# flxrcz/hommx

Hardware: AMD Instinct MI355X
Metric: micro-cell solves/sec (higher is better)
Workload: dtype f64

## Files before the change

### hommx_amd/csrc/fused2d.hip

```cpp
#include <hip/hip_runtime.h>
#include <stdint.h>

#include "kernels.h"
#include "sweep_acc.h"

#ifndef HOMMX_FUSED_WAVES_PER_SIMD
#define HOMMX_FUSED_WAVES_PER_SIMD 2
#endif

namespace hommx {

typedef double d4 __attribute__((ext_vector_type(4)));
typedef double d2 __attribute__((ext_vector_type(2)));

__device__ __forceinline__ double uniform_f64(double v) {
  return __hiloint2double(__builtin_amdgcn_readfirstlane(__double2hiint(v)),
                          __builtin_amdgcn_readfirstlane(__double2loint(v)));
}

struct CoefRow {
  double a0, a1;
  double a0m, a1m;
};

constexpr int MATP = 48;

template <int NB>
struct alignas(16) Lds {
  double mat[(NB + 1) * MATP];
  double ubuf[4 * NB];
  double tsc[16 * 17];
  double rrow[2][NB];
  double vrow[2][NB];
  double vnat[2][NB];
  double e0row[NB];
  double e1row[NB];
  double e0nat[NB];
  double e1nat[NB];
  double dgnat[NB];
  double cenat[NB + 2];
};

template <int NB>
__global__ __launch_bounds__(64, HOMMX_FUSED_WAVES_PER_SIMD) void k_poisson2d_fused(
    const double* __restrict__ coef, const double* __restrict__ Mmat, double* __restrict__ out,
    int32_t* __restrict__ info, int n, long long ncells, const CoefSource src
#ifdef HOMMX_FUSED_DEBUG
    , double* __restrict__ dbg
#endif
) {
  constexpr int NT = NB / 16, KK = NB / 4, CG = 64 / NB;
  constexpr int P = MATP;
  __shared__ Lds<NB> L;

  const long long cell = blockIdx.x;
  if (cell >= ncells) return;
  __builtin_assume(n >= 3);
  __builtin_assume(n <= NB);
  const int l = threadIdx.x;
  const int j = l & 15, k = l >> 4;
  const int c = l % NB, g = l / NB;
  const int lb = l - c;
  const int p0 = NB - n;
  const bool valid = c >= p0;
  const int cn = c - p0;
  const int cm = valid ? (c == p0 ? NB - 1 : c - 1) : c;
  const int cp = valid ? (c == NB - 1 ? p0 : c + 1) : c;
  const int prow = (c & 3) * KK + (c >> 2);

  const int ownB = (k + 1) * P + j;
  int leftB[NT];
#pragma unroll
  for (int tj = 0; tj < NT; ++tj) {
    const int col = 16 * tj + j;
    leftB[tj] = (k + 1) * P + (col == p0 ? NB - 1 : col - 1);
  }
#define OWN(ti, tj, r) (ownB + (16 * (ti) + 4 * (r)) * P + 16 * (tj))
#define LEFT(ti, tj, r) (leftB[tj] + (16 * (ti) + 4 * (r)) * P)
  const unsigned matOff = accl::lds_offset(&L.mat[0]);
  const unsigned haloA = matOff + 8u * (unsigned)(p0 * P + j);

  for (int i = l; i < (NB + 1) * P; i += 64) L.mat[i] = 0.0;
  if (l == 0) L.cenat[0] = 0.0;

  double m00 = 1.0, m01 = 0.0, m10 = 0.0, m11 = 1.0;
  if (Mmat) {
    const double* mp = Mmat + cell * 4;
    m00 = mp[0]; m01 = mp[1]; m10 = mp[2]; m11 = mp[3];
  }
// ... 79 lines not shown
    {
      const double dv = st_diag(rowB, rowA), ov = st_E(rowB, rowA);
      band_write(dv, ov, true, false);
      __syncthreads();
#pragma unroll
      for (int ti = 0; ti < NT; ++ti)
#pragma unroll
        for (int tj = 0; tj <= ti; ++tj)
#pragma unroll
          for (int r = 0; r < 4; ++r) slr[ti][tj][r] = L.mat[OWN(ti, tj, r)];
      __syncthreads();
      band_write(dv, ov, true, true);
      __syncthreads();
    }
    {
      const double dv = st_N(rowB), ov = st_NE(rowB);
      band_write(dv, ov, false, false);
      __syncthreads();
#pragma unroll
      for (int t = 0; t < NT; ++t)
#pragma unroll
        for (int kk = 0; kk < KK; ++kk) wf[t][kk] = L.mat[OWN(kk >> 2, t, kk & 3)];
      __syncthreads();
      band_write(dv, ov, false, true);
      __syncthreads();
    }
    {
      const double dv = -st_diag(cur, rowB), ov = -st_E(cur, rowB);
      band_write(dv, ov, true, false);
      __syncthreads();
#pragma unroll
      for (int ti = 0; ti < NT; ++ti)
#pragma unroll
        for (int tj = 0; tj < NT; ++tj)
#pragma unroll
          for (int r = 0; r < 4; ++r) a[ti][tj][r] = L.mat[OWN(ti, tj, r)];
      __syncthreads();
      band_write(dv, ov, true, true);
      __syncthreads();
    }
    rr[0] = st_p0(cur, rowB); rr[1] = st_p1(cur, rowB);
    rlm = (k >> 1) ? st_p1(rowB, rowA) : st_p0(rowB, rowA);
  }
  double ga_ = 0.0, gb_ = 0.0;
  int bad = 0, badstep = 0;
  double wselR[NT];
#pragma unroll
  for (int tj = 0; tj < NT; ++tj) wselR[tj] = (k == 3 && 16 * tj + j == p0) ? 1.0 : 0.0;
  const double wselC = (j == 15 && k == (p0 & 3)) ? 1.0 : 0.0;
  double indw[KK];
#pragma unroll
  for (int q = 0; q < KK; ++q) indw[q] = uniform_f64((q == (p0 >> 2)) ? 1.0 : 0.0);

  for (int jr = 0; jr <= n - 2; ++jr) {
    const bool lastStep = (jr == n - 2);
    CoefRow nxt = cur;
    if (!lastStep) {
      nxt = load_row(jr + 1);
      asum += nxt.a0 + nxt.a1;
    }
    const double e0c = st_N(cur);
    const double neC = st_NE(cur);
    const double e1c = __shfl(neC, lb + cm, 64);
    if (lastStep) {
      for (int i = l; i < (NB + 1) * P; i += 64) L.mat[i] = 0.0;
      __syncthreads();
      if (g == 0) {
        L.mat[(c + 1) * P + c] = e0c;
        if (valid) L.mat[(c + 1) * P + cp] = neC;
      }
      __syncthreads();
#pragma unroll
      for (int t = 0; t < NT; ++t)
#pragma unroll
        for (int kk = 0; kk < KK; ++kk) wf[t][kk] += L.mat[OWN(kk >> 2, t, kk & 3)];
      __syncthreads();
    }
    const double dgc = st_diag(nxt, cur), cec = st_E(nxt, cur);
    if (g == 0) {
      L.rrow[0][prow] = rr[0];
      L.rrow[1][prow] = rr[1];
      L.e0row[prow] = e0c;
      L.e1row[prow] = e1c;
      L.e0nat[c] = e0c;
      L.e1nat[c] = e1c;
      L.dgnat[c] = dgc;
      L.cenat[1 + c] = cec;
    }

    {
      int badj = 0;
#ifdef HOMMX_FUSED_SWEEP32
      accl::Sweep<NB>::run(a, L.ubuf, j, k, badj);
#else
      __builtin_amdgcn_s_setprio(1);
      if constexpr (NB == 32) accl::block_inverse32(a, L.ubuf, L.tsc, j, k, badj);
      else accl::Sweep<NB>::run(a, L.ubuf, j, k, badj);
      __builtin_amdgcn_s_setprio(0);
#endif
      if (badj && !bad) { bad = 1; badstep = jr + 1; }
    }
#ifdef HOMMX_FUSED_DEBUG
    if (dbg && cell == 0) {
      double* q = dbg + (size_t)jr * 4 * NB * NB;
#pragma unroll
      for (int ti = 0; ti < NT; ++ti)
#pragma unroll
        for (int tj = 0; tj < NT; ++tj)
#pragma unroll
          for (int r = 0; r < 4; ++r) q[(16 * ti + 4 * r + k) * NB + 16 * tj + j] = a[ti][tj][r];
#pragma unroll
      for (int t = 0; t < NT; ++t)
#pragma unroll
        for (int kk = 0; kk < KK; ++kk) q[NB * NB + (16 * t + j) * NB + 4 * kk + k] = wf[t][kk];
    }
#endif

    if (!lastStep) {
#pragma unroll
      for (int ti = 0; ti < NT; ++ti)
#pragma unroll
        for (int tj = 0; tj < NT; ++tj)
#pragma unroll
          for (int r = 0; r < 4; ++r) L.mat[OWN(ti, tj, r)] = a[ti][tj][r];
#pragma unroll
      for (int tj = 0; tj < NT; ++tj)
        accl::masked_lds_store<accl::RowMask<3>::lo, accl::RowMask<3>::hi>(haloA + 128u * tj, a[NT - 1][tj][3]);
    }

    d4 vt[NT][NT];
#pragma unroll
    for (int x = 0; x < NT; ++x)
#pragma unroll
      for (int y = 0; y < NT; ++y) vt[x][y] = d4{0.0, 0.0, 0.0, 0.0};
#pragma unroll
    for (int kk = 0; kk < KK; ++kk)
#pragma unroll
      for (int x = 0; x < NT; ++x)
#pragma unroll
        for (int y = 0; y < NT; ++y)
          vt[x][y] = __builtin_amdgcn_mfma_f64_16x16x4f64(a[kk >> 2][x][kk & 3], wf[y][kk], vt[x][y], 0, 0, 0);

#pragma unroll
    for (int kk = 0; kk < KK; ++kk)
#pragma unroll
      for (int x = 0; x < NT; ++x)
#pragma unroll
        for (int y = 0; y <= x; ++y)
          slr[x][y] = __builtin_amdgcn_mfma_f64_16x16x4f64(vt[kk >> 2][x][kk & 3], wf[y][kk], slr[x][y], 0, 0, 0);

    double z;
    {
      double part[2][NT];
#pragma unroll
      for (int m = 0; m < 2; ++m)
#pragma unroll
        for (int tj = 0; tj < NT; ++tj) part[m][tj] = 0.0;
#pragma unroll
      for (int m = 0; m < 2; ++m)
#pragma unroll
        for (int ti = 0; ti < NT; ++ti) {
          const d4 q = *reinterpret_cast<const d4*>(&L.rrow[m][k * KK + 4 * ti]);
#pragma unroll
          for (int r = 0; r < 4; ++r)
#pragma unroll
            for (int tj = 0; tj < NT; ++tj) part[m][tj] = fma(q[r], a[ti][tj][r], part[m][tj]);
        }
      if (NT == 2) {
        double s_[2];
#pragma unroll
        for (int m = 0; m < 2; ++m) {
          double x = part[m][0], y = part[m][NT - 1];
          swap16(x, y);
          s_[m] = x + y;
        }
        swap32(s_[0], s_[1]);
        z = s_[0] + s_[1];
      } else {
        double x = part[0][0], y = part[1][0];
        swap32(x, y);
        z = add_xor16(x + y);
      }
    }
    ga_ = fma(z, rr[0], ga_);
    gb_ = fma(z, rr[1], gb_);
    L.vnat[k >> 1][c] = z;
    L.vrow[k >> 1][prow] = z;

    {
      double part[2][NT];
#pragma unroll
      for (int m = 0; m < 2; ++m) {
        double v[KK];
#pragma unroll
        for (int q4 = 0; q4 < KK; q4 += 4) {
          const d4 q = *reinterpret_cast<const d4*>(&L.vrow[m][k * KK + q4]);
          v[q4] = q[0]; v[q4 + 1] = q[1]; v[q4 + 2] = q[2]; v[q4 + 3] = q[3];
        }
#pragma unroll
        for (int t = 0; t < NT; ++t) {
          double acc = 0.0;
#pragma unroll
          for (int kk = 0; kk < KK; ++kk) acc = fma(v[kk], wf[t][kk], acc);
          part[m][t] = acc;
        }
      }
      double z6;
      if (NT == 2) {
        double s_[2];
#pragma unroll
        for (int m = 0; m < 2; ++m) {
          double x = part[m][0], y = part[m][NT - 1];
          swap16(x, y);
          s_[m] = x + y;
        }
        swap32(s_[0], s_[1]);
        z6 = s_[0] + s_[1];
      } else {
        double x = part[0][0], y = part[1][0];
        swap32(x, y);
        z6 = add_xor16(x + y);
      }
      rlm += z6;
    }

    if (!lastStep) {
      double e0r[KK], e1r[KK];
#pragma unroll
      for (int q4 = 0; q4 < KK; q4 += 4) {
        const d4 x = *reinterpret_cast<const d4*>(&L.e0row[k * KK + q4]);
        const d4 y = *reinterpret_cast<const d4*>(&L.e1row[k * KK + q4]);
        e0r[q4] = x[0]; e0r[q4 + 1] = x[1]; e0r[q4 + 2] = x[2]; e0r[q4 + 3] = x[3];
        e1r[q4] = y[0]; e1r[q4 + 1] = y[1]; e1r[q4 + 2] = y[2]; e1r[q4 + 3] = y[3];
      }
      {
        double e0q[NT], e1q[NT], dgq[NT], ceq[NT], cemq[NT];
#pragma unroll
        for (int tj = 0; tj < NT; ++tj) {
          e0q[tj] = L.e0nat[16 * tj + j];
          e1q[tj] = L.e1nat[16 * tj + j];
          dgq[tj] = L.dgnat[16 * tj + j];
          ceq[tj] = L.cenat[1 + 16 * tj + j];
          cemq[tj] = L.cenat[16 * tj + j];
        }
#pragma unroll
        for (int ti = 0; ti < NT; ++ti)
#pragma unroll
          for (int r = 0; r < 4; ++r)
#pragma unroll
            for (int tj = 0; tj < NT; ++tj) {
              const double nl = L.mat[LEFT(ti, tj, r)];
              const double nu = L.mat[OWN(ti, tj, r) - P];
              const double nul = L.mat[LEFT(ti, tj, r) - P];
              const double x = fma(e1q[tj], nl, e0q[tj] * a[ti][tj][r]);
              const double xu = fma(e1q[tj], nul, e0q[tj] * nu);
              a[ti][tj][r] = -fma(e0r[4 * ti + r], x, e1r[4 * ti + r] * xu);
            }
#pragma unroll
        for (int t = 0; t < NT; ++t) {
          using namespace accl;
#define DIAG_LO(r) (OneLane<0, 4 * (r)>::lo | OneLane<1, 4 * (r) + 1>::lo | OneLane<2, 4 * (r) + 2>::lo | OneLane<3, 4 * (r) + 3>::lo)
#define DIAG_HI(r) (OneLane<0, 4 * (r)>::hi | OneLane<1, 4 * (r) + 1>::hi | OneLane<2, 4 * (r) + 2>::hi | OneLane<3, 4 * (r) + 3>::hi)
          masked_sub4<DIAG_LO(0), DIAG_HI(0), DIAG_LO(1), DIAG_HI(1), DIAG_LO(2), DIAG_HI(2), DIAG_LO(3), DIAG_HI(3)>(
              a[t][t][0], a[t][t][1], a[t][t][2], a[t][t][3], dgq[t]);
#define SUB_LO(r) (((r) ? OneLane<0, (4 * (r) - 1) & 15>::lo : 0u) | OneLane<1, 4 * (r)>::lo | OneLane<2, 4 * (r) + 1>::lo | OneLane<3, 4 * (r) + 2>::lo)
#define SUB_HI(r) (((r) ? OneLane<0, (4 * (r) - 1) & 15>::hi : 0u) | OneLane<1, 4 * (r)>::hi | OneLane<2, 4 * (r) + 1>::hi | OneLane<3, 4 * (r) + 2>::hi)
          masked_sub4<SUB_LO(0), SUB_HI(0), SUB_LO(1), SUB_HI(1), SUB_LO(2), SUB_HI(2), SUB_LO(3), SUB_HI(3)>(
              a[t][t][0], a[t][t][1], a[t][t][2], a[t][t][3], ceq[t]);
#define SUP_LO(r) (OneLane<0, 4 * (r) + 1>::lo | OneLane<1, 4 * (r) + 2>::lo | OneLane<2, 4 * (r) + 3>::lo | ((r) < 3 ? OneLane<3, (4 * (r) + 4) & 15>::lo : 0u))
#define SUP_HI(r) (OneLane<0, 4 * (r) + 1>::hi | OneLane<1, 4 * (r) + 2>::hi | OneLane<2, 4 * (r) + 3>::hi | ((r) < 3 ? OneLane<3, (4 * (r) + 4) & 15>::hi : 0u))
          masked_sub4<SUP_LO(0), SUP_HI(0), SUP_LO(1), SUP_HI(1), SUP_LO(2), SUP_HI(2), SUP_LO(3), SUP_HI(3)>(
              a[t][t][0], a[t][t][1], a[t][t][2], a[t][t][3], cemq[t]);
#undef DIAG_LO
#undef DIAG_HI
#undef SUB_LO
#undef SUB_HI
#undef SUP_LO
#undef SUP_HI
        }
        if (NT == 2) {
          using namespace accl;
          masked_sub<OneLane<0, 15>::lo, OneLane<0, 15>::hi>(a[NT - 1][0][0], ceq[0]);
          masked_sub<OneLane<3, 0>::lo, OneLane<3, 0>::hi>(a[0][NT - 1][3], cemq[NT - 1]);
        }
        {
          const double cw = readlane_f64(cec, NB - 1);
#pragma unroll
          for (int tj = 0; tj < NT; ++tj) a[NT - 1][tj][3] = fma(-cw, wselR[tj], a[NT - 1][tj][3]);
          const double vcol = -cw * wselC;
#pragma unroll
          for (int ti = 0; ti < NT; ++ti)
#pragma unroll
            for (int r = 0; r < 4; ++r) a[ti][NT - 1][r] = fma(vcol, indw[4 * ti + r], a[ti][NT - 1][r]);
        }
      }

#pragma unroll
      for (int x = 0; x < NT; ++x)
#pragma unroll
        for (int y = 0; y < NT; ++y)
#pragma unroll
          for (int r = 0; r < 4; ++r) L.mat[OWN(x, y, r)] = vt[x][y][r];
#pragma unroll
      for (int y = 0; y < NT; ++y)
        accl::masked_lds_store<accl::RowMask<3>::lo, accl::RowMask<3>::hi>(haloA + 128u * y, vt[NT - 1][y][3]);
#pragma unroll
      for (int t = 0; t < NT; ++t)
#pragma unroll
        for (int kk = 0; kk < KK; ++kk) {
          const double up = L.mat[OWN(kk >> 2, t, kk & 3) - P];
          wf[t][kk] = fma(e1r[kk], up, e0r[kk] * vt[kk >> 2][t][kk & 3]);
        }

      {
        const double v0 = L.vnat[0][c], v1 = L.vnat[1][c];
        const double vm0 = L.vnat[0][cm], vm1 = L.vnat[1][cm];
        rr[0] = fma(vm0, e1c, fma(v0, e0c, st_p0(nxt, cur)));
        rr[1] = fma(vm1, e1c, fma(v1, e0c, st_p1(nxt, cur)));
      }
      cur = nxt;
      __syncthreads();
    }
  }

  {
    if (NT == 2) {
#pragma unroll
      for (int r = 0; r < 4; ++r) L.mat[OWN(1, 0, r)] = slr[NT - 1][0][r];
      __syncthreads();
    }
#pragma unroll
    for (int ti = 0; ti < NT; ++ti)
#pragma unroll
      for (int tj = 0; tj < NT; ++tj)
#pragma unroll
        for (int r = 0; r < 4; ++r) {
          if (tj <= ti) a[ti][tj][r] = -slr[ti][tj][r];
          else a[ti][tj][r] = -L.mat[(16 + j + 1) * P + 4 * r + k];
        }
    {
      using namespace accl;
#pragma unroll
      for (int tj = 0; tj < NT; ++tj) amov<RowMask<3>::lo, RowMask<3>::hi>(a[NT - 1][tj][3], 0.0);
#pragma unroll
      for (int ti = 0; ti < NT; ++ti)
#pragma unroll
        for (int r = 0; r < 4; ++r) amov<ColMask<15>::lo, ColMask<15>::hi>(a[ti][NT - 1][r], 0.0);
      amov<OneLane<3, 15>::lo, OneLane<3, 15>::hi>(a[NT - 1][NT - 1][3], -1.0);
    }
    if (c == NB - 1) rlm = 0.0;
    __syncthreads();
    L.rrow[k >> 1][prow] = rlm;
    L.vnat[k >> 1][c] = rlm;
    __syncthreads();
    int badj = 0;
    accl::Sweep<NB>::run(a, L.ubuf, j, k, badj);
    if (badj && !bad) { bad = 1; badstep = n; }
    double part[2][NT];
#pragma unroll
    for (int m = 0; m < 2; ++m)
#pragma unroll
      for (int tj = 0; tj < NT; ++tj) part[m][tj] = 0.0;
#pragma unroll
    for (int m = 0; m < 2; ++m)
#pragma unroll
      for (int ti = 0; ti < NT; ++ti) {
        const d4 q = *reinterpret_cast<const d4*>(&L.rrow[m][k * KK + 4 * ti]);
#pragma unroll
        for (int r = 0; r < 4; ++r)
#pragma unroll
          for (int tj = 0; tj < NT; ++tj) part[m][tj] = fma(q[r], a[ti][tj][r], part[m][tj]);
      }
    double z;
    if (NT == 2) {
      double s_[2];
#pragma unroll
// ... 12 lines not shown
    ga_ = fma(z, L.vnat[0][c], ga_);
    gb_ = fma(z, L.vnat[1][c], gb_);
  }

  double g00 = (k < 2) ? ga_ : 0.0, g01 = (k < 2) ? gb_ : 0.0, g11 = (k < 2) ? 0.0 : gb_;
#pragma unroll
  for (int off = 32; off >= 1; off >>= 1) {
    g00 += __shfl_xor(g00, off, 64);
    g01 += __shfl_xor(g01, off, 64);
    g11 += __shfl_xor(g11, off, 64);
    asum += __shfl_xor(asum, off, 64);
  }
  if (l == 0) {
    const double h = 1.0 / n;
    constexpr int DUP = 32 / NB;
    const double sc = 0.25 * h * h / DUP;
    const double c0 = 0.5 * h * h * asum / CG;
    const double t00 = m00 * g00 + m01 * g01, t01 = m00 * g01 + m01 * g11;
    const double t10 = m10 * g00 + m11 * g01, t11 = m10 * g01 + m11 * g11;
    double* o = out + cell * 4;
    o[0] = c0 + sc * (t00 * m00 + t01 * m01);
    o[1] = sc * (t00 * m10 + t01 * m11);
    o[2] = sc * (t10 * m00 + t11 * m01);
    o[3] = c0 + sc * (t10 * m10 + t11 * m11);
    if (info) info[cell] = bad ? badstep : 0;
  }
#undef OWN
#undef LEFT
}

hipError_t launch_poisson2d_fused(const double* d_coef, const double* d_M, double* d_out, int32_t* d_info,
                                  int n, long long ncells, hipStream_t stream, CoefSource src) {
  if (ncells <= 0) return hipSuccess;
  dim3 grid((unsigned)ncells), block(64);
#ifndef HOMMX_DEV_LDS_PAD
#define HOMMX_DEV_LDS_PAD 0
#endif
#ifdef HOMMX_FUSED_DEBUG
  extern double* g_fused_dbg;
  if (n <= 16)
    hipLaunchKernelGGL(k_poisson2d_fused<16>, grid, block, 0, stream, d_coef, d_M, d_out, d_info, n, ncells, src, g_fused_dbg);
  else
    hipLaunchKernelGGL(k_poisson2d_fused<32>, grid, block, 0, stream, d_coef, d_M, d_out, d_info, n, ncells, src, g_fused_dbg);
#else
  if (n <= 16)
    hipLaunchKernelGGL(k_poisson2d_fused<16>, grid, block, HOMMX_DEV_LDS_PAD, stream, d_coef, d_M, d_out, d_info, n, ncells, src);
  else
    hipLaunchKernelGGL(k_poisson2d_fused<32>, grid, block, HOMMX_DEV_LDS_PAD, stream, d_coef, d_M, d_out, d_info, n, ncells, src);
#endif
  return hipGetLastError();
}

}
```

### hommx_amd/csrc/sweep_acc.h

```cpp
#pragma once
#include <hip/hip_runtime.h>
#include <stdint.h>

#include "sweep.h"

namespace hommx {
namespace accl {

template <int K> struct RowMask {
  static constexpr unsigned lo = K == 0 ? 0x0000FFFFu : K == 1 ? 0xFFFF0000u : 0u;
  static constexpr unsigned hi = K == 2 ? 0x0000FFFFu : K == 3 ? 0xFFFF0000u : 0u;
};
template <int J> struct ColMask {
  static constexpr unsigned lo = (1u << J) | (1u << (16 + J));
  static constexpr unsigned hi = lo;
};
template <int K, int J> struct OneLane {
  static constexpr int bit = 16 * K + J;
  static constexpr unsigned lo = bit < 32 ? 1u << (bit & 31) : 0u;
  static constexpr unsigned hi = bit >= 32 ? 1u << (bit & 31) : 0u;
};

#define HOMMX_EXEC_SET(LO, HI) "s_mov_b32 exec_lo, %[" LO "]\n\ts_mov_b32 exec_hi, %[" HI "]\n\t"
#define HOMMX_EXEC_ALL "s_mov_b64 exec, -1"
// ... 18 lines not shown
__device__ __forceinline__ void masked_lds_store(unsigned addr, double v) {
  asm volatile(HOMMX_EXEC_SET("lo", "hi") "ds_write_b64 %[a], %[v]\n\t" HOMMX_EXEC_ALL
               : : [a] "v"(addr), [v] "v"(v), [lo] "i"(LO), [hi] "i"(HI) : "memory");
}
template <unsigned LO, unsigned HI>
__device__ __forceinline__ void masked_lds_store2(unsigned addr0, double v0, unsigned addr1, double v1) {
  asm volatile(HOMMX_EXEC_SET("lo", "hi") "ds_write_b64 %[a0], %[v0]\n\tds_write_b64 %[a1], %[v1]\n\t" HOMMX_EXEC_ALL
               : : [a0] "v"(addr0), [v0] "v"(v0), [a1] "v"(addr1), [v1] "v"(v1), [lo] "i"(LO), [hi] "i"(HI) : "memory");
}
template <unsigned RLO, unsigned RHI>
__device__ __forceinline__ void row_rule2(double& a0, double& a1, double w0, double w1) {
  asm(HOMMX_EXEC_SET("rlo", "rhi") "v_mov_b64 %[a0], %[w0]\n\tv_mov_b64 %[a1], %[w1]\n\t" HOMMX_EXEC_ALL
      : [a0] "+v"(a0), [a1] "+v"(a1) : [w0] "v"(w0), [w1] "v"(w1), [rlo] "i"(RLO), [rhi] "i"(RHI));
}
template <unsigned RLO, unsigned RHI>
__device__ __forceinline__ void row_rule1(double& a0, double w0) {
  asm(HOMMX_EXEC_SET("rlo", "rhi") "v_mov_b64 %[a0], %[w0]\n\t" HOMMX_EXEC_ALL : [a0] "+v"(a0) : [w0] "v"(w0), [rlo] "i"(RLO), [rhi] "i"(RHI));
}
template <int R> struct DiagMask {
  static constexpr unsigned lo = OneLane<0, 4 * R>::lo | OneLane<1, 4 * R + 1>::lo | OneLane<2, 4 * R + 2>::lo | OneLane<3, 4 * R + 3>::lo;
  static constexpr unsigned hi = OneLane<0, 4 * R>::hi | OneLane<1, 4 * R + 1>::hi | OneLane<2, 4 * R + 2>::hi | OneLane<3, 4 * R + 3>::hi;
};
__device__ __forceinline__ void diag_plus_one(double& d0, double& d1, double& d2, double& d3) {
  asm(HOMMX_EXEC_SET("l0", "h0") "v_add_f64 %[d0], %[d0], 1.0\n\t" HOMMX_EXEC_SET("l1", "h1") "v_add_f64 %[d1], %[d1], 1.0\n\t"
      HOMMX_EXEC_SET("l2", "h2") "v_add_f64 %[d2], %[d2], 1.0\n\t" HOMMX_EXEC_SET("l3", "h3") "v_add_f64 %[d3], %[d3], 1.0\n\t"
      HOMMX_EXEC_ALL
      : [d0] "+v"(d0), [d1] "+v"(d1), [d2] "+v"(d2), [d3] "+v"(d3)
      : [l0] "i"(DiagMask<0>::lo), [h0] "i"(DiagMask<0>::hi), [l1] "i"(DiagMask<1>::lo), [h1] "i"(DiagMask<1>::hi),
        [l2] "i"(DiagMask<2>::lo), [h2] "i"(DiagMask<2>::hi), [l3] "i"(DiagMask<3>::lo), [h3] "i"(DiagMask<3>::hi));
}

template <class T>
__device__ __forceinline__ unsigned lds_offset(T* p) {
  return (unsigned)(uintptr_t)(__attribute__((address_space(3))) T*)p;
}

__device__ __forceinline__ double readlane_neg_pivot(double v, int lane, unsigned& mn) {
  const int lo = __builtin_amdgcn_readlane(__double2loint(v), lane);
  const int hi = __builtin_amdgcn_readlane(__double2hiint(v), lane);
  const unsigned t = (unsigned)hi + 0x100000u;
  mn = t < mn ? t : mn;
  return __hiloint2double(hi, lo);
}
__device__ __forceinline__ int bad_pivot_min(unsigned mn) { return mn < 0x80200000u; }

#define HOMMX_BC " row_newbcast:%[jk] row_mask:0xf bank_mask:0xf\n\t"
#define HOMMX_PAIR(X, Y) "v_fmac_f64_dpp %[" Y "], %[" X "], %[wo]" HOMMX_BC "v_fmac_f64_dpp %[" X "], %[" X "], %[wk]" HOMMX_BC
#define HOMMX_ONE(X) "v_fmac_f64_dpp %[" X "], %[" X "], %[wk]" HOMMX_BC
#define HOMMX_RCP0 "v_rcp_f64 %[r], %[d]\n\t"
#define HOMMX_RCPE "v_fma_f64 %[e], -%[d], %[r], 1.0\n\t"
#define HOMMX_RCPT "v_fma_f64 %[e], %[e], %[e], %[e]\n\t"
#define HOMMX_RCPR "v_fma_f64 %[r], %[r], %[e], %[r]\n\t"

template <int NB> struct Sweep;

template <>
struct Sweep<32> {
  static constexpr int NB = 32, NT = 2;
  typedef double Mat[2][2][4];

  template <int K>
  static __device__ __forceinline__ void step(Mat& a, double* ubuf, int lk, int j, unsigned& bad, double u0, double u1, double pinv, int npiv) {
    constexpr int tK = K / 16, jK = K % 16, rK = (K % 16) / 4, kK = K % 4, o = 1 - tK;
    constexpr bool more = K + 1 < NB;
    constexpr int K1 = more ? K + 1 : K;
    constexpr int tK1 = K1 / 16, jK1 = K1 % 16, rK1 = (K1 % 16) / 4, kK1 = K1 % 4;
    constexpr int E = tK1 * 4 + rK1;
#define PI(i) ((i) < E ? (i) : (i) + 1)
#define XR(i) a[PI(i) / 4][tK][PI(i) % 4]
#define YR(i) a[PI(i) / 4][o][PI(i) % 4]
    double w[2];
    w[0] = u0 * -pinv;
    w[1] = u1 * -pinv;
    double nu0 = 0.0, nu1 = 0.0, pn = 1.0;
    if constexpr (more) {
      asm volatile("s_nop 1\n\t" HOMMX_PAIR("x", "y")
                   : [x] "+v"(a[tK1][tK][rK1]), [y] "+v"(a[tK1][o][rK1])
                   : [wk] "v"(w[tK]), [wo] "v"(w[o]), [jk] "n"(jK));
      ubuf[lk + j] = a[tK1][0][rK1];
      ubuf[lk + 16 + j] = a[tK1][1][rK1];
      const double dn = readlane_neg_pivot(a[tK1][tK1][rK1], 16 * kK1 + jK1, bad);
      ubuf[NB * kK1 + K1] = dn - 1.0;
      nu0 = ubuf[NB * kK1 + j];
      nu1 = ubuf[NB * kK1 + 16 + j];
      asm volatile("" ::: "memory");
      double e;
      asm volatile(HOMMX_RCP0 HOMMX_PAIR("x0", "y0") HOMMX_PAIR("x1", "y1") HOMMX_RCPE HOMMX_PAIR("x2", "y2")
                       HOMMX_PAIR("x3", "y3") HOMMX_RCPT HOMMX_PAIR("x4", "y4") HOMMX_PAIR("x5", "y5") HOMMX_RCPR
                           HOMMX_PAIR("x6", "y6")
                   : [x0] "+v"(XR(0)), [y0] "+v"(YR(0)), [x1] "+v"(XR(1)), [y1] "+v"(YR(1)), [x2] "+v"(XR(2)), [y2] "+v"(YR(2)),
                     [x3] "+v"(XR(3)), [y3] "+v"(YR(3)), [x4] "+v"(XR(4)), [y4] "+v"(YR(4)), [x5] "+v"(XR(5)), [y5] "+v"(YR(5)),
                     [x6] "+v"(XR(6)), [y6] "+v"(YR(6)), [r] "=&v"(pn), [e] "=&v"(e)
                   : [wk] "v"(w[tK]), [wo] "v"(w[o]), [d] "s"(dn), [jk] "n"(jK));
    } else {
      asm volatile("s_nop 1\n\t" HOMMX_PAIR("x0", "y0") HOMMX_PAIR("x1", "y1") HOMMX_PAIR("x2", "y2") HOMMX_PAIR("x3", "y3")
                       HOMMX_PAIR("x4", "y4") HOMMX_PAIR("x5", "y5") HOMMX_PAIR("x6", "y6") HOMMX_PAIR("x7", "y7")
                   : [x0] "+v"(a[0][tK][0]), [y0] "+v"(a[0][o][0]), [x1] "+v"(a[0][tK][1]), [y1] "+v"(a[0][o][1]),
                     [x2] "+v"(a[0][tK][2]), [y2] "+v"(a[0][o][2]), [x3] "+v"(a[0][tK][3]), [y3] "+v"(a[0][o][3]),
                     [x4] "+v"(a[1][tK][0]), [y4] "+v"(a[1][o][0]), [x5] "+v"(a[1][tK][1]), [y5] "+v"(a[1][o][1]),
                     [x6] "+v"(a[1][tK][2]), [y6] "+v"(a[1][o][2]), [x7] "+v"(a[1][tK][3]), [y7] "+v"(a[1][o][3])
                   : [wk] "v"(w[tK]), [wo] "v"(w[o]), [jk] "n"(jK));
    }
#undef PI
#undef XR
#undef YR
    row_rule2<RowMask<kK>::lo, RowMask<kK>::hi>(a[tK][0][rK], a[tK][1][rK], w[0], w[1]);
    if constexpr (more) {
      if (K + 1 < npiv) step<K + 1>(a, ubuf, lk, j, bad, nu0, nu1, pn, npiv);
    }
  }

  static __device__ __forceinline__ void run(Mat& a, double* ubuf, int j, int k, int& bad, int npiv = NB) {
    const int lk = NB * k;
    ubuf[lk + j] = a[0][0][0];
    ubuf[lk + 16 + j] = a[0][1][0];
    unsigned b = 0xffffffffu;
    const double d0 = readlane_neg_pivot(a[0][0][0], 0, b);
    ubuf[0] = d0 - 1.0;
    const double u0 = ubuf[j], u1 = ubuf[16 + j];
    step<0>(a, ubuf, lk, j, b, u0, u1, fast_rcp(d0), npiv);
    diag_plus_one(a[0][0][0], a[0][0][1], a[0][0][2], a[0][0][3]);
    diag_plus_one(a[1][1][0], a[1][1][1], a[1][1][2], a[1][1][3]);
    bad |= bad_pivot_min(b);
  }
};

template <>
struct Sweep<16> {
  static constexpr int NB = 16, NT = 1;
  typedef double Mat[1][1][4];

  template <int K>
  static __device__ __forceinline__ void step(Mat& a, double* ubuf, int lk, int j, unsigned& bad, double u0, double pinv, int npiv) {
    constexpr int jK = K, rK = K / 4, kK = K % 4;
    constexpr bool more = K + 1 < NB;
    constexpr int K1 = more ? K + 1 : K;
    constexpr int jK1 = K1, rK1 = K1 / 4, kK1 = K1 % 4;
#define PI(i) ((i) < rK1 ? (i) : (i) + 1)
    const double w = u0 * -pinv;
    double nu0 = 0.0, pn = 1.0;
    if constexpr (more) {
      asm volatile("s_nop 1\n\t" HOMMX_ONE("x") : [x] "+v"(a[0][0][rK1]) : [wk] "v"(w), [jk] "n"(jK));
      ubuf[lk + j] = a[0][0][rK1];
      const double dn = readlane_neg_pivot(a[0][0][rK1], 16 * kK1 + jK1, bad);
      ubuf[NB * kK1 + K1] = dn - 1.0;
      nu0 = ubuf[NB * kK1 + j];
      asm volatile("" ::: "memory");
      double e;
      asm volatile(HOMMX_RCP0 HOMMX_ONE("x0") HOMMX_RCPE HOMMX_ONE("x1") HOMMX_RCPT HOMMX_ONE("x2") HOMMX_RCPR
                   : [x0] "+v"(a[0][0][PI(0)]), [x1] "+v"(a[0][0][PI(1)]), [x2] "+v"(a[0][0][PI(2)]), [r] "=&v"(pn), [e] "=&v"(e)
                   : [wk] "v"(w), [d] "s"(dn), [jk] "n"(jK));
    } else {
      asm volatile("s_nop 1\n\t" HOMMX_ONE("x0") HOMMX_ONE("x1") HOMMX_ONE("x2") HOMMX_ONE("x3")
                   : [x0] "+v"(a[0][0][0]), [x1] "+v"(a[0][0][1]), [x2] "+v"(a[0][0][2]), [x3] "+v"(a[0][0][3])
                   : [wk] "v"(w), [jk] "n"(jK));
    }
#undef PI
#ifdef HOMMX_ROW_RULE_EXEC
    row_rule1<RowMask<kK>::lo, RowMask<kK>::hi>(a[0][0][rK], w);
#else
    a[0][0][rK] = (lk == NB * kK) ? w : a[0][0][rK];
#endif
    if constexpr (more) {
      if (K + 1 < npiv) step<K + 1>(a, ubuf, lk, j, bad, nu0, pn, npiv);
    }
  }

  static __device__ __forceinline__ void run(Mat& a, double* ubuf, int j, int k, int& bad, int npiv = NB) {
    const int lk = NB * k;
    ubuf[lk + j] = a[0][0][0];
    unsigned b = 0xffffffffu;
    const double d0 = readlane_neg_pivot(a[0][0][0], 0, b);
    ubuf[0] = d0 - 1.0;
    const double u0 = ubuf[j];
    step<0>(a, ubuf, lk, j, b, u0, fast_rcp(d0), npiv);
    diag_plus_one(a[0][0][0], a[0][0][1], a[0][0][2], a[0][0][3]);
    bad |= bad_pivot_min(b);
  }
};

typedef double v4d __attribute__((ext_vector_type(4)));
__device__ __forceinline__ v4d transpose_tile(v4d x, double* tsc, int j, int k) {
#pragma unroll
  for (int r = 0; r < 4; ++r) tsc[(4 * r + k) * 17 + j] = x[r];
  __builtin_amdgcn_fence(__ATOMIC_RELEASE, "wavefront");
  __builtin_amdgcn_wave_barrier();
  __builtin_amdgcn_fence(__ATOMIC_ACQUIRE, "wavefront");
  v4d y;
#pragma unroll
  for (int r = 0; r < 4; ++r) y[r] = tsc[j * 17 + 4 * r + k];
  __builtin_amdgcn_wave_barrier();
  return y;
}
__device__ __forceinline__ void block_inverse32(double (&a)[2][2][4], double* ubuf, double* tsc, int j, int k, int& bad, int npiv = 32) {
  auto mm = [](double x, double y, v4d c) { return __builtin_amdgcn_mfma_f64_16x16x4f64(x, y, c, 0, 0, 0); };
  double t00[1][1][4], sc[1][1][4], nu[4];
#pragma unroll
  for (int r = 0; r < 4; ++r) { t00[0][0][r] = a[0][0][r]; nu[r] = -a[0][1][r]; }
  Sweep<16>::run(t00, ubuf, j, k, bad);
  v4d nxt = v4d{0.0, 0.0, 0.0, 0.0};
#pragma unroll
  for (int q = 0; q < 4; ++q) nxt = mm(t00[0][0][q], nu[q], nxt);
  const v4d nx = transpose_tile(nxt, tsc, j, k);
  {
    v4d c = v4d{a[1][1][0], a[1][1][1], a[1][1][2], a[1][1][3]};
#pragma unroll
    for (int q = 0; q < 4; ++q) c = mm(nxt[q], a[0][1][q], c);
#pragma unroll
    for (int r = 0; r < 4; ++r) sc[0][0][r] = c[r];
  }
  Sweep<16>::run(sc, ubuf, j, k, bad, npiv - 16);
  v4d n21 = v4d{0.0, 0.0, 0.0, 0.0};
#pragma unroll
  for (int q = 0; q < 4; ++q) n21 = mm(sc[0][0][q], nx[q], n21);
  v4d n11 = v4d{t00[0][0][0], t00[0][0][1], t00[0][0][2], t00[0][0][3]};
#pragma unroll
  for (int q = 0; q < 4; ++q) n11 = mm(nx[q], n21[q], n11);
  const v4d n12 = transpose_tile(n21, tsc, j, k);
#pragma unroll
  for (int r = 0; r < 4; ++r) {
    a[0][0][r] = n11[r];
    a[0][1][r] = n12[r];
    a[1][0][r] = n21[r];
    a[1][1][r] = sc[0][0][r];
  }
}

}
}
```

Baseline: 7.034 million.

## Interleave previous step's arrow MFMAs into the next step's serial pivot sweep

Moves the per-step vt/slr MFMA products, which depend on the previous step's inverse, so they run one step later inside the latency-bound sweep of the next block inverse. The ops go in through a hook called at each pivot slot, fenced with sched_barrier. The wf update, the rlm update and the e-row loads are deferred to match, and the e-row LDS buffers are double-buffered, with a final drain after the loop. The aim is to hide MFMA work behind the serial rcp/FMA chain of the sweep, at the cost of higher register pressure from keeping np, vt and two e-row copies live. Optional clock64 profiling instrumentation is also added behind a macro.

Measured after the change: 6.911 million. -1.8%, worse.

```diff
diff --git a/hommx_amd/csrc/fused2d.hip b/hommx_amd/csrc/fused2d.hip
--- a/hommx_amd/csrc/fused2d.hip
+++ b/hommx_amd/csrc/fused2d.hip
@@ -24,6 +24,59 @@
 };
 
 constexpr int MATP = 48;
+
+enum { FP_HEAD, FP_SWEEP_A, FP_INV_MFMA, FP_SWEEP_B, FP_ARROW, FP_SPARSE, FP_BARRIER, FP_STEPS, FP_N };
+#ifdef HOMMX_FUSED_PROF
+__device__ long long g_fused_prof[FP_N];
+#define FP_T(i) do { const long long now_ = clock64(); pt_[i] += now_ - t_last_; t_last_ = now_; } while (0)
+#else
+#define FP_T(i) do { } while (0)
+#endif
+template <int NB>
+struct ArrowHook {
+  static constexpr int NT = NB / 16, KK = NB / 4;
+  static constexpr int N3 = KK * NT * NT, N4 = KK * NT * (NT + 1) / 2, NI = N3 + N4;
+  const double (&np)[NT][NT][4];
+  const double (&wf)[NT][KK];
+  d4 (&vt)[NT][NT];
+  d4 (&slr)[NT][NT];
+  const bool on;
+#ifdef HOMMX_FUSED_PROF
+  long long* pt_;
+  long long& t_last_;
+#endif
+  template <int I>
+  __device__ __forceinline__ void item() {
+    if constexpr (I < N3) {
+      constexpr int kk = I / (NT * NT), x = (I / NT) % NT, y = I % NT;
+      vt[x][y] = __builtin_amdgcn_mfma_f64_16x16x4f64(np[kk >> 2][x][kk & 3], wf[y][kk], vt[x][y], 0, 0, 0);
+    } else {
+      constexpr int PER = NT * (NT + 1) / 2, kk = (I - N3) / PER, q = (I - N3) % PER;
+      constexpr int x = q == 0 ? 0 : 1, y = q == 2 ? 1 : 0;
+      slr[x][y] = __builtin_amdgcn_mfma_f64_16x16x4f64(vt[kk >> 2][x][kk & 3], wf[y][kk], slr[x][y], 0, 0, 0);
+    }
+  }
+  template <int I0, int I1>
+  __device__ __forceinline__ void items() {
+    if constexpr (I0 < I1) {
+      item<I0>();
+      items<I0 + 1, I1>();
+    }
+  }
+  template <int S>
+  __device__ __forceinline__ void slot() {
+    constexpr int I0 = NI * S / NB, I1 = NI * (S + 1) / NB;
+    if constexpr (I0 < I1) {
+      if (on) {
+        __builtin_amdgcn_sched_barrier(0);
+        items<I0, I1>();
+        __builtin_amdgcn_sched_barrier(0);
+      }
+    }
+  }
+  __device__ __forceinline__ void drain() { items<0, NI>(); }
+  template <int P> __device__ __forceinline__ void mark() { FP_T(FP_SWEEP_A + P); }
+};
 
 template <int NB>
 struct alignas(16) Lds {
@@ -33,8 +86,8 @@
   double rrow[2][NB];
   double vrow[2][NB];
   double vnat[2][NB];
-  double e0row[NB];
-  double e1row[NB];
+  double e0row[2][NB];
+  double e1row[2][NB];
   double e0nat[NB];
   double e1nat[NB];
   double dgnat[NB];
@@ -220,8 +273,65 @@
 #pragma unroll
   for (int q = 0; q < KK; ++q) indw[q] = uniform_f64((q == (p0 >> 2)) ? 1.0 : 0.0);
 
+#ifdef HOMMX_FUSED_PROF
+  long long pt_[FP_N] = {};
+  long long t_last_ = clock64();
+#endif
+#define LOAD_EROWS(PB)                                                                        \
+  double e0r[KK], e1r[KK];                                                                    \
+  _Pragma("unroll") for (int q4 = 0; q4 < KK; q4 += 4) {                                      \
+    const d4 x = *reinterpret_cast<const d4*>(&L.e0row[PB][k * KK + q4]);                     \
+    const d4 y = *reinterpret_cast<const d4*>(&L.e1row[PB][k * KK + q4]);                     \
+    e0r[q4] = x[0]; e0r[q4 + 1] = x[1]; e0r[q4 + 2] = x[2]; e0r[q4 + 3] = x[3];               \
+    e1r[q4] = y[0]; e1r[q4 + 1] = y[1]; e1r[q4 + 2] = y[2]; e1r[q4 + 3] = y[3];               \
+  }
+  double np[NT][NT][4];
+#pragma unroll
+  for (int ti = 0; ti < NT; ++ti)
+#pragma unroll
+    for (int tj = 0; tj < NT; ++tj)
+#pragma unroll
+      for (int r = 0; r < 4; ++r) np[ti][tj][r] = 0.0;
+  auto rlast_update = [&]() {
+    double part[2][NT];
+#pragma unroll
+    for (int m = 0; m < 2; ++m) {
+      double v[KK];
+#pragma unroll
+      for (int q4 = 0; q4 < KK; q4 += 4) {
+        const d4 q = *reinterpret_cast<const d4*>(&L.vrow[m][k * KK + q4]);
+        v[q4] = q[0]; v[q4 + 1] = q[1]; v[q4 + 2] = q[2]; v[q4 + 3] = q[3];
+      }
+#pragma unroll
+      for (int t = 0; t < NT; ++t) {
+        double acc = 0.0;
+#pragma unroll
+        for (int kk = 0; kk < KK; ++kk) acc = fma(v[kk], wf[t][kk], acc);
+        part[m][t] = acc;
+      }
+    }
+    double z6;
+    if (NT == 2) {
+      double s_[2];
+#pragma unroll
+      for (int m = 0; m < 2; ++m) {
+        double x = part[m][0], y = part[m][NT - 1];
+        swap16(x, y);
+        s_[m] = x + y;
+      }
+      swap32(s_[0], s_[1]);
+      z6 = s_[0] + s_[1];
+    } else {
+      double x = part[0][0], y = part[1][0];
+      swap32(x, y);
+      z6 = add_xor16(x + y);
+    }
+    rlm += z6;
+  };
   for (int jr = 0; jr <= n - 2; ++jr) {
     const bool lastStep = (jr == n - 2);
+    const bool pending = jr > 0;
+    const int pb = jr & 1;
     CoefRow nxt = cur;
     if (!lastStep) {
       nxt = load_row(jr + 1);
@@ -230,44 +340,42 @@
     const double e0c = st_N(cur);
     const double neC = st_NE(cur);
     const double e1c = __shfl(neC, lb + cm, 64);
-    if (lastStep) {
-      for (int i = l; i < (NB + 1) * P; i += 64) L.mat[i] = 0.0;
-      __syncthreads();
-      if (g == 0) {
-        L.mat[(c + 1) * P + c] = e0c;
-        if (valid) L.mat[(c + 1) * P + cp] = neC;
-      }
-      __syncthreads();
-#pragma unroll
-      for (int t = 0; t < NT; ++t)
-#pragma unroll
-        for (int kk = 0; kk < KK; ++kk) wf[t][kk] += L.mat[OWN(kk >> 2, t, kk & 3)];
-      __syncthreads();
-    }
     const double dgc = st_diag(nxt, cur), cec = st_E(nxt, cur);
     if (g == 0) {
       L.rrow[0][prow] = rr[0];
       L.rrow[1][prow] = rr[1];
-      L.e0row[prow] = e0c;
-      L.e1row[prow] = e1c;
+      L.e0row[pb][prow] = e0c;
+      L.e1row[pb][prow] = e1c;
       L.e0nat[c] = e0c;
       L.e1nat[c] = e1c;
       L.dgnat[c] = dgc;
       L.cenat[1 + c] = cec;
     }
 
+    d4 vt[NT][NT];
+#pragma unroll
+    for (int x = 0; x < NT; ++x)
+#pragma unroll
+      for (int y = 0; y < NT; ++y) vt[x][y] = d4{0.0, 0.0, 0.0, 0.0};
+#ifdef HOMMX_FUSED_PROF
+    ArrowHook<NB> ihook{np, wf, vt, slr, pending, pt_, t_last_};
+#else
+    ArrowHook<NB> ihook{np, wf, vt, slr, pending};
+#endif
+    FP_T(FP_HEAD);
     {
       int badj = 0;
 #ifdef HOMMX_FUSED_SWEEP32
-      accl::Sweep<NB>::run(a, L.ubuf, j, k, badj);
+      accl::Sweep<NB>::run(a, L.ubuf, j, k, badj, NB, ihook);
 #else
       __builtin_amdgcn_s_setprio(1);
-      if constexpr (NB == 32) accl::block_inverse32(a, L.ubuf, L.tsc, j, k, badj);
-      else accl::Sweep<NB>::run(a, L.ubuf, j, k, badj);
+      if constexpr (NB == 32) accl::block_inverse32(a, L.ubuf, L.tsc, j, k, badj, NB, ihook);
+      else accl::Sweep<NB>::run(a, L.ubuf, j, k, badj, NB, ihook);
       __builtin_amdgcn_s_setprio(0);
 #endif
       if (badj && !bad) { bad = 1; badstep = jr + 1; }
     }
+    FP_T(NB == 32 ? FP_INV_MFMA : FP_SWEEP_A);
 #ifdef HOMMX_FUSED_DEBUG
     if (dbg && cell == 0) {
       double* q = dbg + (size_t)jr * 4 * NB * NB;
@@ -277,12 +385,58 @@
         for (int tj = 0; tj < NT; ++tj)
 #pragma unroll
           for (int r = 0; r < 4; ++r) q[(16 * ti + 4 * r + k) * NB + 16 * tj + j] = a[ti][tj][r];
+    }
+#endif
+
+    if (pending) {
+      rlast_update();
+      LOAD_EROWS(pb ^ 1)
+#pragma unroll
+      for (int x = 0; x < NT; ++x)
+#pragma unroll
+        for (int y = 0; y < NT; ++y)
+#pragma unroll
+          for (int r = 0; r < 4; ++r) L.mat[OWN(x, y, r)] = vt[x][y][r];
+#pragma unroll
+      for (int y = 0; y < NT; ++y)
+        accl::masked_lds_store<accl::RowMask<3>::lo, accl::RowMask<3>::hi>(haloA + 128u * y, vt[NT - 1][y][3]);
 #pragma unroll
       for (int t = 0; t < NT; ++t)
 #pragma unroll
+        for (int kk = 0; kk < KK; ++kk) {
+          const double up = L.mat[OWN(kk >> 2, t, kk & 3) - P];
+          wf[t][kk] = fma(e1r[kk], up, e0r[kk] * vt[kk >> 2][t][kk & 3]);
+        }
+    }
+    if (lastStep) {
+      for (int i = l; i < (NB + 1) * P; i += 64) L.mat[i] = 0.0;
+      __syncthreads();
+      if (g == 0) {
+        L.mat[(c + 1) * P + c] = e0c;
+        if (valid) L.mat[(c + 1) * P + cp] = neC;
+      }
+      __syncthreads();
+#pragma unroll
+      for (int t = 0; t < NT; ++t)
+#pragma unroll
+        for (int kk = 0; kk < KK; ++kk) wf[t][kk] += L.mat[OWN(kk >> 2, t, kk & 3)];
+      __syncthreads();
+    }
+#ifdef HOMMX_FUSED_DEBUG
+    if (dbg && cell == 0) {
+      double* q = dbg + (size_t)jr * 4 * NB * NB;
+#pragma unroll
+      for (int t = 0; t < NT; ++t)
+#pragma unroll
         for (int kk = 0; kk < KK; ++kk) q[NB * NB + (16 * t + j) * NB + 4 * kk + k] = wf[t][kk];
     }
 #endif
+#pragma unroll
+    for (int ti = 0; ti < NT; ++ti)
+#pragma unroll
+      for (int tj = 0; tj < NT; ++tj)
+#pragma unroll
+        for (int r = 0; r < 4; ++r) np[ti][tj][r] = a[ti][tj][r];
 
     if (!lastStep) {
 #pragma unroll
@@ -295,27 +449,6 @@
       for (int tj = 0; tj < NT; ++tj)
         accl::masked_lds_store<accl::RowMask<3>::lo, accl::RowMask<3>::hi>(haloA + 128u * tj, a[NT - 1][tj][3]);
     }
-
-    d4 vt[NT][NT];
-#pragma unroll
-    for (int x = 0; x < NT; ++x)
-#pragma unroll
-      for (int y = 0; y < NT; ++y) vt[x][y] = d4{0.0, 0.0, 0.0, 0.0};
-#pragma unroll
-    for (int kk = 0; kk < KK; ++kk)
-#pragma unroll
-      for (int x = 0; x < NT; ++x)
-#pragma unroll
-        for (int y = 0; y < NT; ++y)
-          vt[x][y] = __builtin_amdgcn_mfma_f64_16x16x4f64(a[kk >> 2][x][kk & 3], wf[y][kk], vt[x][y], 0, 0, 0);
-
-#pragma unroll
-    for (int kk = 0; kk < KK; ++kk)
-#pragma unroll
-      for (int x = 0; x < NT; ++x)
-#pragma unroll
-        for (int y = 0; y <= x; ++y)
-          slr[x][y] = __builtin_amdgcn_mfma_f64_16x16x4f64(vt[kk >> 2][x][kk & 3], wf[y][kk], slr[x][y], 0, 0, 0);
 
     double z;
     {
@@ -355,52 +488,8 @@
     L.vnat[k >> 1][c] = z;
     L.vrow[k >> 1][prow] = z;
 
-    {
-      double part[2][NT];
-#pragma unroll
-      for (int m = 0; m < 2; ++m) {
-        double v[KK];
-#pragma unroll
-        for (int q4 = 0; q4 < KK; q4 += 4) {
-          const d4 q = *reinterpret_cast<const d4*>(&L.vrow[m][k * KK + q4]);
-          v[q4] = q[0]; v[q4 + 1] = q[1]; v[q4 + 2] = q[2]; v[q4 + 3] = q[3];
-        }
-#pragma unroll
-        for (int t = 0; t < NT; ++t) {
-          double acc = 0.0;
-#pragma unroll
-          for (int kk = 0; kk < KK; ++kk) acc = fma(v[kk], wf[t][kk], acc);
-          part[m][t] = acc;
-        }
-      }
-      double z6;
-      if (NT == 2) {
-        double s_[2];
-#pragma unroll
-        for (int m = 0; m < 2; ++m) {
-          double x = part[m][0], y = part[m][NT - 1];
-          swap16(x, y);
-          s_[m] = x + y;
-        }
-        swap32(s_[0], s_[1]);
-        z6 = s_[0] + s_[1];
-      } else {
-        double x = part[0][0], y = part[1][0];
-        swap32(x, y);
-        z6 = add_xor16(x + y);
-      }
-      rlm += z6;
-    }
-
     if (!lastStep) {
-      double e0r[KK], e1r[KK];
-#pragma unroll
-      for (int q4 = 0; q4 < KK; q4 += 4) {
-        const d4 x = *reinterpret_cast<const d4*>(&L.e0row[k * KK + q4]);
-        const d4 y = *reinterpret_cast<const d4*>(&L.e1row[k * KK + q4]);
-        e0r[q4] = x[0]; e0r[q4 + 1] = x[1]; e0r[q4 + 2] = x[2]; e0r[q4 + 3] = x[3];
-        e1r[q4] = y[0]; e1r[q4 + 1] = y[1]; e1r[q4 + 2] = y[2]; e1r[q4 + 3] = y[3];
-      }
+      LOAD_EROWS(pb)
       {
         double e0q[NT], e1q[NT], dgq[NT], ceq[NT], cemq[NT];
 #pragma unroll
@@ -463,23 +552,6 @@
         }
       }
 
-#pragma unroll
-      for (int x = 0; x < NT; ++x)
-#pragma unroll
-        for (int y = 0; y < NT; ++y)
-#pragma unroll
-          for (int r = 0; r < 4; ++r) L.mat[OWN(x, y, r)] = vt[x][y][r];
-#pragma unroll
-      for (int y = 0; y < NT; ++y)
-        accl::masked_lds_store<accl::RowMask<3>::lo, accl::RowMask<3>::hi>(haloA + 128u * y, vt[NT - 1][y][3]);
-#pragma unroll
-      for (int t = 0; t < NT; ++t)
-#pragma unroll
-        for (int kk = 0; kk < KK; ++kk) {
-          const double up = L.mat[OWN(kk >> 2, t, kk & 3) - P];
-          wf[t][kk] = fma(e1r[kk], up, e0r[kk] * vt[kk >> 2][t][kk & 3]);
-        }
-
       {
         const double v0 = L.vnat[0][c], v1 = L.vnat[1][c];
         const double vm0 = L.vnat[0][cm], vm1 = L.vnat[1][cm];
@@ -487,9 +559,34 @@
         rr[1] = fma(vm1, e1c, fma(v1, e0c, st_p1(nxt, cur)));
       }
       cur = nxt;
-      __syncthreads();
-    }
-  }
+      FP_T(FP_SPARSE);
+      __syncthreads();
+      FP_T(FP_BARRIER);
+    }
+  }
+  {
+    FP_T(FP_SPARSE);
+    d4 vt[NT][NT];
+#pragma unroll
+    for (int x = 0; x < NT; ++x)
+#pragma unroll
+      for (int y = 0; y < NT; ++y) vt[x][y] = d4{0.0, 0.0, 0.0, 0.0};
+#ifdef HOMMX_FUSED_PROF
+    ArrowHook<NB> ihook{np, wf, vt, slr, true, pt_, t_last_};
+#else
+    ArrowHook<NB> ihook{np, wf, vt, slr, true};
+#endif
+    ihook.drain();
+    FP_T(FP_ARROW);
+    rlast_update();
+  }
+#undef LOAD_EROWS
+#ifdef HOMMX_FUSED_PROF
+  FP_T(FP_SPARSE);
+  pt_[FP_STEPS] = n - 1;
+  if (cell == 0 && l == 0)
+    for (int i = 0; i < FP_N; ++i) g_fused_prof[i] += pt_[i];
+#endif
 
   {
     if (NT == 2) {
@@ -608,3 +705,13 @@
 }
 
 }
+
+#ifdef HOMMX_FUSED_PROF
+extern "C" void hommx_fused_prof_read(long long* out, int reset) {
+  (void)hipMemcpyFromSymbol(out, HIP_SYMBOL(hommx::g_fused_prof), sizeof(long long) * hommx::FP_N);
+  if (reset) {
+    long long z[hommx::FP_N] = {};
+    (void)hipMemcpyToSymbol(HIP_SYMBOL(hommx::g_fused_prof), z, sizeof(z));
+  }
+}
+#endif
diff --git a/hommx_amd/csrc/sweep_acc.h b/hommx_amd/csrc/sweep_acc.h
--- a/hommx_amd/csrc/sweep_acc.h
+++ b/hommx_amd/csrc/sweep_acc.h
@@ -94,6 +94,16 @@
 #define HOMMX_RCPT "v_fma_f64 %[e], %[e], %[e], %[e]\n\t"
 #define HOMMX_RCPR "v_fma_f64 %[r], %[r], %[e], %[r]\n\t"
 
+struct NoHook {
+  template <int S> __device__ __forceinline__ void slot() {}
+  template <int P> __device__ __forceinline__ void mark() {}
+};
+template <class H, int BASE>
+struct ShiftedHook {
+  H& h;
+  template <int S> __device__ __forceinline__ void slot() { h.template slot<BASE + S>(); }
+};
+
 template <int NB> struct Sweep;
 
 template <>
@@ -101,8 +111,8 @@
   static constexpr int NB = 32, NT = 2;
   typedef double Mat[2][2][4];
 
-  template <int K>
-  static __device__ __forceinline__ void step(Mat& a, double* ubuf, int lk, int j, unsigned& bad, double u0, double u1, double pinv, int npiv) {
+  template <int K, class H>
+  static __device__ __forceinline__ void step(Mat& a, double* ubuf, int lk, int j, unsigned& bad, double u0, double u1, double pinv, int npiv, H& h) {
     constexpr int tK = K / 16, jK = K % 16, rK = (K % 16) / 4, kK = K % 4, o = 1 - tK;
     constexpr bool more = K + 1 < NB;
     constexpr int K1 = more ? K + 1 : K;
@@ -126,6 +136,7 @@
       nu0 = ubuf[NB * kK1 + j];
       nu1 = ubuf[NB * kK1 + 16 + j];
       asm volatile("" ::: "memory");
+      h.template slot<K>();
       double e;
       asm volatile(HOMMX_RCP0 HOMMX_PAIR("x0", "y0") HOMMX_PAIR("x1", "y1") HOMMX_RCPE HOMMX_PAIR("x2", "y2")
                        HOMMX_PAIR("x3", "y3") HOMMX_RCPT HOMMX_PAIR("x4", "y4") HOMMX_PAIR("x5", "y5") HOMMX_RCPR
@@ -135,6 +146,7 @@
                      [x6] "+v"(XR(6)), [y6] "+v"(YR(6)), [r] "=&v"(pn), [e] "=&v"(e)
                    : [wk] "v"(w[tK]), [wo] "v"(w[o]), [d] "s"(dn), [jk] "n"(jK));
     } else {
+      h.template slot<K>();
       asm volatile("s_nop 1\n\t" HOMMX_PAIR("x0", "y0") HOMMX_PAIR("x1", "y1") HOMMX_PAIR("x2", "y2") HOMMX_PAIR("x3", "y3")
                        HOMMX_PAIR("x4", "y4") HOMMX_PAIR("x5", "y5") HOMMX_PAIR("x6", "y6") HOMMX_PAIR("x7", "y7")
                    : [x0] "+v"(a[0][tK][0]), [y0] "+v"(a[0][o][0]), [x1] "+v"(a[0][tK][1]), [y1] "+v"(a[0][o][1]),
@@ -148,11 +160,12 @@
 #undef YR
     row_rule2<RowMask<kK>::lo, RowMask<kK>::hi>(a[tK][0][rK], a[tK][1][rK], w[0], w[1]);
     if constexpr (more) {
-      if (K + 1 < npiv) step<K + 1>(a, ubuf, lk, j, bad, nu0, nu1, pn, npiv);
+      if (K + 1 < npiv) step<K + 1>(a, ubuf, lk, j, bad, nu0, nu1, pn, npiv, h);
     }
   }
 
-  static __device__ __forceinline__ void run(Mat& a, double* ubuf, int j, int k, int& bad, int npiv = NB) {
+  template <class H>
+  static __device__ __forceinline__ void run(Mat& a, double* ubuf, int j, int k, int& bad, int npiv, H& h) {
     const int lk = NB * k;
     ubuf[lk + j] = a[0][0][0];
     ubuf[lk + 16 + j] = a[0][1][0];
@@ -160,10 +173,14 @@
     const double d0 = readlane_neg_pivot(a[0][0][0], 0, b);
     ubuf[0] = d0 - 1.0;
     const double u0 = ubuf[j], u1 = ubuf[16 + j];
-    step<0>(a, ubuf, lk, j, b, u0, u1, fast_rcp(d0), npiv);
+    step<0>(a, ubuf, lk, j, b, u0, u1, fast_rcp(d0), npiv, h);
     diag_plus_one(a[0][0][0], a[0][0][1], a[0][0][2], a[0][0][3]);
     diag_plus_one(a[1][1][0], a[1][1][1], a[1][1][2], a[1][1][3]);
     bad |= bad_pivot_min(b);
+  }
+  static __device__ __forceinline__ void run(Mat& a, double* ubuf, int j, int k, int& bad, int npiv = NB) {
+    NoHook h;
+    run(a, ubuf, j, k, bad, npiv, h);
   }
 };
 
@@ -172,8 +189,8 @@
   static constexpr int NB = 16, NT = 1;
   typedef double Mat[1][1][4];
 
-  template <int K>
-  static __device__ __forceinline__ void step(Mat& a, double* ubuf, int lk, int j, unsigned& bad, double u0, double pinv, int npiv) {
+  template <int K, class H>
+  static __device__ __forceinline__ void step(Mat& a, double* ubuf, int lk, int j, unsigned& bad, double u0, double pinv, int npiv, H& h) {
     constexpr int jK = K, rK = K / 4, kK = K % 4;
     constexpr bool more = K + 1 < NB;
     constexpr int K1 = more ? K + 1 : K;
@@ -188,11 +205,13 @@
       ubuf[NB * kK1 + K1] = dn - 1.0;
       nu0 = ubuf[NB * kK1 + j];
       asm volatile("" ::: "memory");
+      h.template slot<K>();
       double e;
       asm volatile(HOMMX_RCP0 HOMMX_ONE("x0") HOMMX_RCPE HOMMX_ONE("x1") HOMMX_RCPT HOMMX_ONE("x2") HOMMX_RCPR
                    : [x0] "+v"(a[0][0][PI(0)]), [x1] "+v"(a[0][0][PI(1)]), [x2] "+v"(a[0][0][PI(2)]), [r] "=&v"(pn), [e] "=&v"(e)
                    : [wk] "v"(w), [d] "s"(dn), [jk] "n"(jK));
     } else {
+      h.template slot<K>();
       asm volatile("s_nop 1\n\t" HOMMX_ONE("x0") HOMMX_ONE("x1") HOMMX_ONE("x2") HOMMX_ONE("x3")
                    : [x0] "+v"(a[0][0][0]), [x1] "+v"(a[0][0][1]), [x2] "+v"(a[0][0][2]), [x3] "+v"(a[0][0][3])
                    : [wk] "v"(w), [jk] "n"(jK));
@@ -204,20 +223,25 @@
     a[0][0][rK] = (lk == NB * kK) ? w : a[0][0][rK];
 #endif
     if constexpr (more) {
-      if (K + 1 < npiv) step<K + 1>(a, ubuf, lk, j, bad, nu0, pn, npiv);
+      if (K + 1 < npiv) step<K + 1>(a, ubuf, lk, j, bad, nu0, pn, npiv, h);
     }
   }
 
-  static __device__ __forceinline__ void run(Mat& a, double* ubuf, int j, int k, int& bad, int npiv = NB) {
+  template <class H>
+  static __device__ __forceinline__ void run(Mat& a, double* ubuf, int j, int k, int& bad, int npiv, H& h) {
     const int lk = NB * k;
     ubuf[lk + j] = a[0][0][0];
     unsigned b = 0xffffffffu;
     const double d0 = readlane_neg_pivot(a[0][0][0], 0, b);
     ubuf[0] = d0 - 1.0;
     const double u0 = ubuf[j];
-    step<0>(a, ubuf, lk, j, b, u0, fast_rcp(d0), npiv);
+    step<0>(a, ubuf, lk, j, b, u0, fast_rcp(d0), npiv, h);
     diag_plus_one(a[0][0][0], a[0][0][1], a[0][0][2], a[0][0][3]);
     bad |= bad_pivot_min(b);
+  }
+  static __device__ __forceinline__ void run(Mat& a, double* ubuf, int j, int k, int& bad, int npiv = NB) {
+    NoHook h;
+    run(a, ubuf, j, k, bad, npiv, h);
   }
 };
 
@@ -234,12 +258,16 @@
   __builtin_amdgcn_wave_barrier();
   return y;
 }
-__device__ __forceinline__ void block_inverse32(double (&a)[2][2][4], double* ubuf, double* tsc, int j, int k, int& bad, int npiv = 32) {
+template <class H>
+__device__ __forceinline__ void block_inverse32(double (&a)[2][2][4], double* ubuf, double* tsc, int j, int k, int& bad, int npiv, H& h) {
+  ShiftedHook<H, 0> hA{h};
+  ShiftedHook<H, 16> hB{h};
   auto mm = [](double x, double y, v4d c) { return __builtin_amdgcn_mfma_f64_16x16x4f64(x, y, c, 0, 0, 0); };
   double t00[1][1][4], sc[1][1][4], nu[4];
 #pragma unroll
   for (int r = 0; r < 4; ++r) { t00[0][0][r] = a[0][0][r]; nu[r] = -a[0][1][r]; }
-  Sweep<16>::run(t00, ubuf, j, k, bad);
+  Sweep<16>::run(t00, ubuf, j, k, bad, 16, hA);
+  h.template mark<0>();
   v4d nxt = v4d{0.0, 0.0, 0.0, 0.0};
 #pragma unroll
   for (int q = 0; q < 4; ++q) nxt = mm(t00[0][0][q], nu[q], nxt);
@@ -251,7 +279,9 @@
 #pragma unroll
     for (int r = 0; r < 4; ++r) sc[0][0][r] = c[r];
   }
-  Sweep<16>::run(sc, ubuf, j, k, bad, npiv - 16);
+  h.template mark<1>();
+  Sweep<16>::run(sc, ubuf, j, k, bad, npiv - 16, hB);
+  h.template mark<2>();
   v4d n21 = v4d{0.0, 0.0, 0.0, 0.0};
 #pragma unroll
   for (int q = 0; q < 4; ++q) n21 = mm(sc[0][0][q], nx[q], n21);
@@ -267,6 +297,10 @@
     a[1][1][r] = sc[0][0][r];
   }
 }
-
-}
-}
+__device__ __forceinline__ void block_inverse32(double (&a)[2][2][4], double* ubuf, double* tsc, int j, int k, int& bad, int npiv = 32) {
+  NoHook h;
+  block_inverse32(a, ubuf, tsc, j, k, bad, npiv, h);
+}
+
+}
+}
```
